# ctlab/metafast

Measured on AMD Instinct MI355X. Metric: k-mers/s counted+graphed at k=31, 150 bp reads, higher is better.
Workload: dtype u64

## Files before the change

metafast_amd/csrc/mf_common.h:

```cpp
#pragma once
#include <hip/hip_runtime.h>
#include <stdint.h>
#include <stdarg.h>
#include <stdio.h>
#include <string.h>
#include <map>
#include <string>
#include <vector>
#include "../../include/metafast_hip.h"

int mf_set_error(const char *fmt, ...);

#define MF_HIP(call)                                                                              \
    do {                                                                                          \
        hipError_t e__ = (call);                                                                  \
        if (e__ != hipSuccess)                                                                    \
            return mf_set_error("%s failed: %s (%s:%d)", #call, hipGetErrorString(e__), __FILE__, \
                                __LINE__);                                                        \
    } while (0)
#define MF_TRY(call)                  \
    do {                              \
        int r__ = (call);             \
        if (r__ < 0) return r__;      \
    } while (0)
// ... 54 lines not shown
    int64_t opt_device_parse = 1;
    int64_t opt_device_parse_piece = 8 << 20, opt_device_parse_threads = 8;
    int64_t opt_device_parse_min = 1 << 20;
    int64_t opt_host_pinned = 0;
    int64_t opt_file_cache_gb = 0;
    int64_t opt_gz_device_min = 32 << 20;
    int64_t opt_gz_piece = 2 << 20;
    int64_t opt_ut_double_after = 4;
    int64_t opt_ut_plain_rounds = 3;
    int64_t opt_cc_compress = 1;
    int64_t opt_stream_count = 1;
    int64_t opt_stream_count_min = 512 << 20, opt_stream_count_piece = 256 << 20;
    int64_t opt_stream_count_test_pct = 100;
    uint64_t n_streamed = 0, n_stream_stepped_back = 0;
    void *up_stream = nullptr;
    int64_t opt_wide_skm = 1;
    int64_t opt_wide_skm_min = 1 << 20;
    int64_t opt_wide_skm_lazy_order = 1;
    int64_t opt_wide_skm_fine = 8;
    int64_t opt_wide_skm_pack = 1;
    int64_t opt_wide_skm_merge = 1;
    int64_t opt_wide_skm_lead = 1;
    int64_t opt_wide_skm_unit = 2400;
    int64_t opt_wide_finish = 1;
    int64_t opt_wide_big_bucket = 256;
    int64_t opt_wide_distinct = 1280;
    int64_t opt_wide_ablate = 0;
    int64_t opt_wide_passes = 0;
    int64_t opt_cc_sparse = 1;
    int64_t opt_stats_slices = 0;
    int64_t opt_dcc_sparse = 0;
    int64_t opt_dcc_test_fail = 0; int64_t dcc_test_calls[3] = {0, 0, 0};
    int64_t opt_nbr_global = 0;
    int64_t opt_scatter_fast = 1;
    int64_t opt_ablate = 0;
    struct span { size_t off, sz; };
    struct region { char *base; size_t size; std::vector<span> free_spans; };
    std::vector<region> regions;
    std::vector<struct mf_file_entry *> file_cache; size_t file_cache_bytes = 0; uint64_t file_cache_clock = 0;
    size_t arena_bytes = 0;
    uint64_t n_slice_restarts = 0, n_dparse_files = 0, n_dparse_stepped_back = 0, n_wide_big = 0, n_wide_hashed = 0, n_ut_doubled = 0, n_pilots = 0, n_gz_device = 0;
    std::vector<mf_timer_rec> pending;
    std::vector<hipEvent_t> event_pool;
    struct ktime { int64_t n = 0; double total_ms = 0, max_ms = 0; };
    std::map<std::string, ktime> timings;
};

int  mf_alloc(mf_ctx *ctx, size_t bytes, void **out);
void mf_release(mf_ctx *ctx, void *p, size_t bytes);
size_t mf_arena_idle(const mf_ctx *ctx);
int  mf_collect_timers(mf_ctx *ctx);
int  mf_debug_sync(mf_ctx *ctx, const char *what);
#define MF_DBG(ctx, what) do { if ((ctx)->opt_verbose >= 2) MF_TRY(mf_debug_sync((ctx), (what))); } while (0)

struct mf_ktimer {
    mf_ctx *ctx; int idx;
    mf_ktimer(mf_ctx *c, const char *name);
    ~mf_ktimer();
};

struct mf_range {
    bool on;
    explicit mf_range(const char *name);
    ~mf_range();
};

// ... 452 lines not shown
```

metafast_amd/csrc/mf_ctx.hip:

```cpp
#include "mf_common.h"
#include <time.h>
#include <stdlib.h>

static thread_local char g_err[1024] = "";

int mf_set_error(const char *fmt, ...) {
    va_list ap;
    va_start(ap, fmt);
    vsnprintf(g_err, sizeof g_err, fmt, ap);
    va_end(ap);
    return MF_ERR;
}

extern "C" const char *mf_last_error(void) { return g_err; }

#include <dlfcn.h>
#include <mutex>
static int (*g_roctx_push)(const char *) = nullptr;
static int (*g_roctx_pop)(void) = nullptr;
static bool roctx_ready() {
    static std::once_flag once;
    std::call_once(once, [] {
        const char *want = getenv("MF_ROCTX");
        if (want ? atoi(want) == 0 : getenv("ROCP_TOOL_LIBRARIES") == nullptr) return;
// ... 155 lines not shown
    else if (s == "wide_skm_merge") ctx->opt_wide_skm_merge = v;
    else if (s == "wide_skm_pack") ctx->opt_wide_skm_pack = v;
    else if (s == "wide_skm_fine") ctx->opt_wide_skm_fine = v;
    else if (s == "wide_skm_lazy_order") ctx->opt_wide_skm_lazy_order = v;
    else if (s == "dcc_sparse") ctx->opt_dcc_sparse = v;
    else if (s == "dcc_test_fail") { ctx->opt_dcc_test_fail = v; ctx->dcc_test_calls[1] = ctx->dcc_test_calls[2] = 0; }
    else if (s == "cc_sparse") ctx->opt_cc_sparse = v;
    else if (s == "stats_slices") { if (v < 0 || v > 4096) return mf_set_error("stats_slices must be in [0, 4096]"); ctx->opt_stats_slices = v; }
    else if (s == "gz_device_min_bytes") ctx->opt_gz_device_min = v;
    else if (s == "gz_piece_bytes") { if (v < 4096) return mf_set_error("gz_piece_bytes must be at least 4096"); ctx->opt_gz_piece = v; }
    else if (s == "ut_double_after") { if (v < 1 || v > 64) return mf_set_error("ut_double_after must be in [1, 64]"); ctx->opt_ut_double_after = v; }
    else if (s == "wide_finish") ctx->opt_wide_finish = v ? 1 : 0;
    else if (s == "wide_big_bucket") { if (v < 1 || v > 256) return mf_set_error("wide_big_bucket must be in [1, 256]"); ctx->opt_wide_big_bucket = v; }
    else if (s == "wide_ablate") ctx->opt_wide_ablate = v;
    else if (s == "wide_distinct") { if (v < 1 || v > 1280) return mf_set_error("wide_distinct must be in [1, 1280]"); ctx->opt_wide_distinct = v; }
    else if (s == "wide_passes") { if (v < 0 || v > 65536) return mf_set_error("wide_passes must be in [0, 65536]"); ctx->opt_wide_passes = v; }
    else if (s == "file_cache") {
        if (v < 0) { size_t fr = 0, tot = 0; MF_HIP(hipSetDevice(ctx->device)); MF_HIP(hipMemGetInfo(&fr, &tot)); v = std::max<int64_t>(1, (int64_t)(tot >> 32) / -v); }
        ctx->opt_file_cache_gb = v;
        if (!v) mf_file_cache_clear(ctx);
    }
    else if (s == "skm_pilot") ctx->opt_skm_pilot = v;
    else if (s == "device_parse") ctx->opt_device_parse = v;
    else if (s == "device_parse_min_bytes") ctx->opt_device_parse_min = v;
    else if (s == "device_parse_piece_bytes") ctx->opt_device_parse_piece = v;
    else if (s == "device_parse_threads") ctx->opt_device_parse_threads = v;
    else if (s == "host_pinned") ctx->opt_host_pinned = v;
    else if (s == "skm_dynq") ctx->opt_skm_dynq = v;
    else if (s == "part_good") { if (v < 16 || v > 4096) return mf_set_error("part_good out of [16,4096]"); ctx->opt_part_good = v; }
    else if (s == "unit_parts_long") { if (v < 0 || v > 4) return mf_set_error("unit_parts_long out of [0,4]"); ctx->opt_unit_parts_long = v; }
    else if (s == "skm_unit_records") { if (v != 0 && (v < 64 || v > (1 << 20))) return mf_set_error("skm_unit_records out of [64,2^20] (0: by k)"); ctx->opt_skm_unit_records = v; }
    else if (s == "skm_unit_distinct") { if (v < 64 || v > 3400) return mf_set_error("skm_unit_distinct out of [64,3400]"); ctx->opt_skm_unit_distinct = v; }
    else if (s == "union_samples") ctx->opt_union_samples = v;
    else return mf_set_error("unknown option '%s'", name);
    return MF_OK;
}

extern "C" int64_t mf_ctx_stat(mf_ctx *ctx, const char *name) {
    if (!ctx || !name) return mf_set_error("mf_ctx_stat: NULL argument");
    const std::string s(name);
    if (s == "slice_restarts") return (int64_t)ctx->n_slice_restarts;
    if (s == "gz_files_inflated_into_hbm") return (int64_t)ctx->n_gz_device;
    if (s == "pilot_runs") return (int64_t)ctx->n_pilots;
    if (s == "unitig_doublings") return (int64_t)ctx->n_ut_doubled;
    if (s == "wide_big_entries") return (int64_t)ctx->n_wide_big;
    if (s == "wide_hashed_entries") return (int64_t)ctx->n_wide_hashed;
    if (s == "streamed_counts") return (int64_t)ctx->n_streamed;
    if (s == "streamed_counts_stepped_back") return (int64_t)ctx->n_stream_stepped_back;
    if (s == "device_parsed_files") return (int64_t)ctx->n_dparse_files;
    if (s == "device_parser_stepped_back") return (int64_t)ctx->n_dparse_stepped_back;
    if (s == "hipmalloc_calls") return (int64_t)ctx->n_hipmalloc;
    if (s == "hipmalloc_bytes") return (int64_t)ctx->b_hipmalloc;
    if (s == "hipmalloc_us") return (int64_t)(ctx->t_hipmalloc * 1e6);
    if (s == "arena_bytes") return (int64_t)ctx->arena_bytes;
    if (s == "arena_idle_bytes") return (int64_t)mf_arena_idle(ctx);
    return mf_set_error("mf_ctx_stat: unknown name '%s'", name);
}
extern "C" int mf_ctx_synchronize(mf_ctx *ctx) {
    if (!ctx) return mf_set_error("ctx is NULL");
    MF_HIP(hipStreamSynchronize(ctx->stream));
    return MF_OK;
}

static const size_t MF_ALIGN = 256;
static bool arena_take(mf_ctx *ctx, size_t bytes, void **out, bool spare_big) {
    int br = -1, bs = -1; size_t best = ~(size_t)0;
    for (size_t r = 0; r < ctx->regions.size(); r++)
        for (size_t s = 0; s < ctx->regions[r].free_spans.size(); s++) {
            size_t sz = ctx->regions[r].free_spans[s].sz;
            if (spare_big && sz >= ((size_t)48 << 30) && sz / 4 >= bytes) continue;
            if (sz >= bytes && sz < best) { best = sz; br = (int)r; bs = (int)s; }
        }
    if (br < 0) return false;
    auto &R = ctx->regions[br];
    mf_ctx::span sp = R.free_spans[bs];
    *out = R.base + sp.off;
// ... 133 lines not shown
```

metafast_amd/csrc/mf_skm.hip:

```cpp
#include "mf_common.h"
#include "mf_count_dev.h"
#include <algorithm>
#include <memory>
#include <vector>

typedef ulonglong2 skm_rec;
typedef uint32_t skm_v4 __attribute__((ext_vector_type(4)));
#define SKM_LINE 4
#define SKM_QCAP 16
#define SKM_DIGIT_BITS 22
#ifdef SKM_BIG_UNITS
#define SKM_CT 1024
#elif defined(SKM_SMALL_UNITS)
#define SKM_CT 256
#else
#define SKM_CT 512
#endif
#define SKM_NW (SKM_CT / 64)

__device__ __forceinline__ bool skm_rec_valid(const skm_rec &r) { return ((uint32_t)r.y & 63u) != 63u; }
__device__ __forceinline__ uint32_t skm_rec_n(const skm_rec &r) { return (uint32_t)r.y & 63u; }
__device__ __forceinline__ uint32_t skm_rec_digits(const skm_rec &r) { return (uint32_t)(r.y >> 6) & ((1u << SKM_DIGIT_BITS) - 1u); }

template <int K> struct skm_word {
// ... 188 lines not shown
};
__device__ __forceinline__ skm_stage skm_stage_carve(unsigned char *smem, int nd) {
    skm_stage L;
    L.nd = nd;
    L.line = reinterpret_cast<skm_rec *>(smem);
    L.cur = reinterpret_cast<uint64_t *>(L.line + (size_t)nd * SKM_LINE + 64);
    L.q_pos = L.cur + nd;
    L.ctr = reinterpret_cast<uint32_t *>(L.q_pos + 16 * SKM_QCAP);
    L.q_d = L.ctr + nd + 64;
    return L;
}
__host__ __device__ static inline size_t skm_stage_bytes(int nd) {
    return ((size_t)nd * SKM_LINE + 64) * 16 + (size_t)nd * 8 + 16 * SKM_QCAP * 8 + ((size_t)nd + 64) * 4 + 16 * SKM_QCAP * 4;
}
__device__ __forceinline__ void skm_lds_write4_add_rtn4(const uint32_t (&wa)[4], const skm_v4 (&wv)[4], const uint32_t (&a)[4],
                                                        const uint32_t (&inc)[4], uint32_t (&old)[4]) {
    asm volatile("ds_write_b128 %4, %8\n\tds_write_b128 %5, %9\n\tds_write_b128 %6, %10\n\tds_write_b128 %7, %11\n\t"
                 "ds_add_rtn_u32 %0, %12, %16\n\tds_add_rtn_u32 %1, %13, %17\n\tds_add_rtn_u32 %2, %14, %18\n\t"
                 "ds_add_rtn_u32 %3, %15, %19\n\ts_waitcnt lgkmcnt(0)"
                 : "=&v"(old[0]), "=&v"(old[1]), "=&v"(old[2]), "=&v"(old[3])
                 : "v"(wa[0]), "v"(wa[1]), "v"(wa[2]), "v"(wa[3]), "v"(wv[0]), "v"(wv[1]), "v"(wv[2]), "v"(wv[3]),
                   "v"(a[0]), "v"(a[1]), "v"(a[2]), "v"(a[3]), "v"(inc[0]), "v"(inc[1]), "v"(inc[2]), "v"(inc[3])
                 : "memory");
}
#define SKM_CH 256
#define SKM_NONE (~0ull)
struct skm_dyn {
    unsigned long long *gcur;
    const uint64_t *rend;
    unsigned int *overflow;
    uint64_t dump;
    unsigned long long *save;
};
template <bool DYN>
__device__ __forceinline__ uint64_t skm_take_line(const skm_stage &L, uint32_t dg, const skm_dyn &Dy) {
    uint64_t pos = L.cur[dg];
    if (DYN && (pos == SKM_NONE || (pos & (uint64_t)(SKM_CH - 1)) == 0ull)) {
        pos = atomicAdd(&Dy.gcur[dg], (unsigned long long)SKM_CH);
        if (pos + SKM_CH > Dy.rend[dg]) { atomicExch(Dy.overflow, 1u); pos = Dy.dump; }
    }
    L.cur[dg] = pos + SKM_LINE;
    return pos;
}
template <bool DYN = false>
__device__ __forceinline__ void skm_stage_insert(const skm_stage &L, skm_rec *__restrict__ out, const uint32_t (&d)[4],
                                                 const skm_rec (&rec)[4], bool (&pending)[4], const skm_dyn &Dy = skm_dyn()) {
    const uint32_t ctr0 = mf_lds_addr(L.ctr), line0 = mf_lds_addr(L.line);
    const uint32_t dummy_ctr = ctr0 + 4u * ((uint32_t)L.nd + (uint32_t)mf_lane());
    const uint32_t dummy_slot = line0 + 16u * ((uint32_t)L.nd * SKM_LINE + (uint32_t)mf_lane());
    skm_v4 wv[4];
#pragma unroll
    for (int b = 0; b < 4; b++) { wv[b].x = (uint32_t)rec[b].x; wv[b].y = (uint32_t)(rec[b].x >> 32); wv[b].z = (uint32_t)rec[b].y; wv[b].w = (uint32_t)(rec[b].y >> 32); }
    for (;;) {
        bool any = false;
#pragma unroll
        for (int b = 0; b < 4; b++) any |= pending[b];
        if (__ballot(any) == 0ull) break;
        uint32_t ca[4], w[4], inc[4], old[4], old2[4], wa[4];
        bool got[4];
#pragma unroll
        for (int b = 0; b < 4; b++) ca[b] = pending[b] ? ctr0 + 4u * d[b] : dummy_ctr;
        mf_lds_read4(ca, w);
#pragma unroll
        for (int b = 0; b < 4; b++) inc[b] = (pending[b] && (w[b] & 0xFFFFu) < (uint32_t)SKM_LINE) ? 1u : 0u;
        mf_lds_add_rtn4(ca, inc, old);
#pragma unroll
        for (int b = 0; b < 4; b++) {
            got[b] = inc[b] && (old[b] & 0xFFFFu) < (uint32_t)SKM_LINE;
            wa[b] = got[b] ? line0 + 16u * (d[b] * SKM_LINE + (old[b] & 0xFFFFu)) : dummy_slot;
            ca[b] = got[b] ? ctr0 + 4u * d[b] : dummy_ctr;
            inc[b] = got[b] ? 0x10000u : 0u;
        }
        skm_lds_write4_add_rtn4(wa, wv, ca, inc, old2);
        uint64_t *qpos = L.q_pos + (threadIdx.x >> 6) * SKM_QCAP;
        uint32_t *qd = L.q_d + (threadIdx.x >> 6) * SKM_QCAP;
        const uint64_t lt_mask = (1ull << mf_lane()) - 1ull;
#pragma unroll
        for (int b = 0; b < 4; b++) {
            const bool fl = got[b] && (old2[b] >> 16) == (uint32_t)(SKM_LINE - 1);
            const unsigned long long F = __ballot(fl);
            if (got[b]) pending[b] = false;
            if (F == 0ull) continue;
            const uint32_t n = (uint32_t)__popcll(F), qi = (uint32_t)__popcll(F & lt_mask);
            uint64_t mypos = 0;
            if (fl) mypos = skm_take_line<DYN>(L, d[b], Dy);
            for (uint32_t e0 = 0; e0 < n; e0 += SKM_QCAP) {
                if (fl && qi >= e0 && qi < e0 + SKM_QCAP) { qpos[qi - e0] = mypos; qd[qi - e0] = d[b]; }
                asm volatile("s_waitcnt lgkmcnt(0)" ::: "memory");
                const uint32_t e = e0 + ((uint32_t)mf_lane() >> 2), c = (uint32_t)mf_lane() & 3u;
                if (e < n) {
                    const uint32_t dd = qd[e - e0];
                    const uint64_t pp = qpos[e - e0];
                    const skm_rec v = L.line[dd * SKM_LINE + c];
                    out[pp + c] = v;
                    asm volatile("" ::: "memory");
                    if (c == 0) __hip_atomic_store(&L.ctr[dd], 0u, __ATOMIC_RELEASE, MF_WG);
                }
                asm volatile("s_waitcnt lgkmcnt(0)" ::: "memory");
            }
        }
        asm volatile("" ::: "memory");
        __builtin_amdgcn_wave_barrier();
    }
}
template <bool DYN = false>
__device__ __forceinline__ void skm_stage_flush_all(const skm_stage &L, skm_rec *__restrict__ out, int nd, const skm_dyn &Dy = skm_dyn()) {
    const skm_rec SENT = make_ulonglong2(~0ull, ~0ull);
    for (int d = threadIdx.x; d < nd; d += blockDim.x) {
        const uint32_t c = L.ctr[d] >> 16;
        if (c) {
            const uint64_t pos = skm_take_line<DYN>(L, (uint32_t)d, Dy);
            for (uint32_t s = 0; s < (uint32_t)SKM_LINE; s++) out[pos + s] = s < c ? L.line[d * SKM_LINE + s] : SENT;
            L.ctr[d] = 0;
        }
        if (DYN) {
            uint64_t pos = L.cur[d];
            if (Dy.save) Dy.save[(size_t)blockIdx.x * nd + d] = pos;
            else if (pos != SKM_NONE) for (; (pos & (uint64_t)(SKM_CH - 1)) != 0ull; pos++) out[pos] = SENT;
        }
    }
}
__global__ void k_skm_close_chunks(const unsigned long long *__restrict__ save, uint64_t n, uint64_t cap, skm_rec *__restrict__ out) {
    const uint64_t i = (uint64_t)blockIdx.x * blockDim.x + threadIdx.x;
    if (i >= n) return;
    uint64_t pos = save[i];
    if (pos == SKM_NONE || pos >= cap) return;
    const skm_rec SENT = make_ulonglong2(~0ull, ~0ull);
    for (; (pos & (uint64_t)(SKM_CH - 1)) != 0ull; pos++) out[pos] = SENT;
}

#define SKM_LCAP 384
#define SKM_FAST_WAVE_BYTES (64 * 16 + 64 * 8 + (SKM_LCAP + 1) * 8)
template <int K, bool DYN, bool FAST>
__global__ __launch_bounds__(1024) void k_skm_scatter(const uint8_t *__restrict__ bases, uint64_t n_bases, const uint32_t *__restrict__ vmask,
                                                      uint64_t n_words, uint64_t words_per_block, int bits1,
                                                      const uint64_t *__restrict__ blockstart, int G, skm_rec *__restrict__ out, skm_dyn Dy,
                                                      uint32_t dlo, uint32_t dhi) {
    extern __shared__ __attribute__((aligned(16))) unsigned char smem[];
    const int nd = 1 << bits1;
    skm_stage L = skm_stage_carve(smem, nd);
    if (DYN) Dy.dump += (uint64_t)blockIdx.x * SKM_CH;
    for (int i = threadIdx.x; i < nd; i += blockDim.x) {
        L.cur[i] = DYN ? (Dy.save ? (uint64_t)Dy.save[(size_t)blockIdx.x * nd + i] : SKM_NONE) : blockstart[(size_t)i * G + blockIdx.x];
        L.ctr[i] = 0;
    }
// ... 171 lines not shown
            for (int dd = 32; dd >= 1; dd >>= 1) raw += __shfl_down(raw, dd, 64);
            if (mf_lane() == 0 && raw) atomicAdd(n_valid, (unsigned long long)raw);
        }
        uint32_t tot;
        uint32_t ex = mf_block_excl_scan(mine, scratch, &tot);
        for (int j = 0; j < ipt; j++) {
            const int b = b0 + j;
            if (b < nd) {
                const uint32_t c = (L.ctr[b] + 3u) & ~3u;
                L.cur[b] = obase + ex;
                ostart[(size_t)p * nd + b] = obase + ex;
                olen[(size_t)p * nd + b] = c;
                if (oocc) oocc[(size_t)p * nd + b] = occ[b];
                ex += c;
            }
        }
        __syncthreads();
        for (int i = threadIdx.x; i < nd; i += blockDim.x) L.ctr[i] = 0;
        if (threadIdx.x < 64) L.ctr[nd + threadIdx.x] = 0;
        __syncthreads();
        for (uint32_t jb = 0; jb < len; jb += 4 * blockDim.x) {
            skm_rec v[4]; uint32_t d[4]; bool pend[4];
#pragma unroll
            for (int u = 0; u < 4; u++) {
                const uint32_t j = jb + u * blockDim.x + threadIdx.x;
                v[u] = j < len ? src[j] : make_ulonglong2(~0ull, ~0ull);
                pend[u] = skm_rec_valid(v[u]);
                d[u] = pend[u] ? ((skm_rec_digits(v[u]) >> shift) & dmask) : 0u;
            }
            skm_stage_insert(L, out, d, v, pend);
        }
        __syncthreads();
        skm_stage_flush_all(L, out, nd);
        __syncthreads();
    }
}

#define SKM_MAX_PASSES 64
__device__ __forceinline__ uint32_t skm_pass_of(uint64_t key) {
    uint32_t g = ((uint32_t)(key >> 32) * 0xC2B2AE35u) ^ ((uint32_t)key * 0x27D4EB2Fu);
    g ^= g >> 15; g *= 0x165667B1u;
    return g >> 24;
}

#ifdef SKM_BIG_UNITS
#define C2_SLOTS 8192
#define C2_FILL 6800
#define C2_WG_PER_CU 1
#elif defined(SKM_SMALL_UNITS)
#define C2_SLOTS 2048
#define C2_FILL 1700
#define C2_WG_PER_CU 3
#else
#define C2_WG_PER_CU 2
#define C2_SLOTS 4096
#define C2_FILL 3400
#endif
#define C2_QN 128
#define C2_LH 64
#define C2_ITEMS 848
#define C2_W 2
#define DD_BITS (SKM_CT > 512 ? 12 : 11)
#define C2_DD 4
static constexpr size_t C2_LDS = (size_t)C2_SLOTS * 12 + (size_t)SKM_CT * 16 + (size_t)(SKM_CT / 64) * (C2_ITEMS * 2 + C2_QN * 8 + C2_QN * 2) + 2 * C2_LH * 4 + 48;
static_assert(C2_LDS <= 160 * 1024 / C2_WG_PER_CU, "workgroups per CU");

// ... 939 lines not shown
            int Bc = 0; while (Bc < 30 && (double)(1ull << Bc) < want_units) Bc++;
            const int r = std::max(1, std::min(Bc - bits1, std::min((int)SKM_DIGIT_BITS, 30 - bits1)));
            if (ctx->opt_verbose) fprintf(stderr, "[mf] skm pilot: %.4f distinct k-mers per occurrence -> %d bits after level 1 (planned from the occurrences alone: %d)\n", rho, r, total_bits - bits1);
            lv.resize(1);
            if (r <= MF_MAX_DIGIT_BITS) lv.push_back(r); else { lv.push_back((r + 1) / 2); lv.push_back(r / 2); }
            total_bits = 0; for (int b : lv) total_bits += b;
            if (kthr >= 0 && kept >= 0.0 && !A.doff.p) {
                const double per_unit = (double)n_occ * kept / (double)(1ull << total_bits);
                int sb = 0; while (sb < 4 && per_unit / (double)(1 << sb) > (double)ctx->opt_part_good) sb++;
                A.split_bits = sb; split_from_pilot = true;
                if (ctx->opt_verbose) fprintf(stderr, "[mf] skm pilot: %.4f k-mers per occurrence survive the cut: %.0f per counting unit -> %d table partition(s) per unit\n", kept, per_unit, 1 << sb);
            }
        }
    }
    if (!A.doff.p) {
        if (!split_from_pilot) A.split_bits = A.table_bits > 0 ? std::max(0, std::min(4, A.table_bits - total_bits)) : 1;
        if (total_bits + A.split_bits > 30) A.split_bits = 30 - total_bits;
        A.np_total = (uint32_t)(1ull << (total_bits + A.split_bits));
        MF_TRY(A.doff.alloc(ctx, (size_t)A.np_total + 1));
    }
    MF_HIP(hipMemsetAsync(&scal[6], 0, 8, st));
    headroom = false;
    const unsigned long long cap_l1 = cap, cap_last = final_cap(cap);
    if (dlo != 0 || dhi != (uint32_t)nd1) {
        np = dhi - dlo;
        mf_buf<uint64_t> ps; MF_TRY(ps.alloc(ctx, np)); mf_buf<uint32_t> pl, po; MF_TRY(pl.alloc(ctx, np)); MF_TRY(po.alloc(ctx, np));
        MF_HIP(hipMemcpyAsync(ps.p, pstart.p + dlo, (size_t)np * 8, hipMemcpyDeviceToDevice, st));
        MF_HIP(hipMemcpyAsync(pl.p, plen.p + dlo, (size_t)np * 4, hipMemcpyDeviceToDevice, st));
        MF_HIP(hipMemcpyAsync(po.p, pocc.p + dlo, (size_t)np * 4, hipMemcpyDeviceToDevice, st));
        pstart.swap(ps); plen.swap(pl); pocc.swap(po);
    }
    int used = 0;
    mf_buf<skm_rec> spare;
    for (size_t li = 1; li < lv.size(); li++) {
        const int bits = lv[li], nd = 1 << bits;
        const uint64_t cap2 = cap + (uint64_t)np * SKM_LINE * nd;
        const uint64_t np2 = (uint64_t)np * nd;
        if (np2 > 0xFFFFFFF0ull) return mf_set_error("too many partitions");
        const bool last = li + 1 == lv.size();
        mf_buf<skm_rec> bufB;
        if (spare.p && spare.n >= cap2) bufB.swap(spare);
        else if (bufB.alloc(ctx, std::max<unsigned long long>(cap2, cap_last)) != MF_OK) {
            if (ctx->opt_verbose) fprintf(stderr, "[mf] skm: no room for %.1f GB of level-%zu records (arena %.1f GB): %s\n", cap2 * 16 / 1e9, li + 1, ctx->arena_bytes / 1e9, mf_last_error());
            return MF_SKM_NOMEM;
        }
        mf_buf<uint64_t> ostart; MF_TRY(ostart.alloc(ctx, np2));
        mf_buf<uint32_t> olen; MF_TRY(olen.alloc(ctx, np2));
        mf_buf<uint32_t> oocc; if (last) MF_TRY(oocc.alloc(ctx, np2));
        const size_t lds = skm_stage_bytes(nd);
        const unsigned grid = (unsigned)std::min<uint64_t>(np, (uint64_t)ctx->n_cu * (lds > 72 * 1024 ? 1 : 2));
        {
            MF_TRY(skm_set_lds(k_skm_split, lds));
            mf_ktimer t(ctx, "k_skm_split");
            k_skm_split<<<grid, 1024, lds, st>>>(bufA.p, pstart.p, plen.p, np, SKM_DIGIT_BITS - used - bits, bits, bufB.p, ostart.p, olen.p, oocc.p,
                                                 li == 1 ? &scal[6] : nullptr, li == 1 ? rebase : 0);
        }
        MF_DBG(ctx, "k_skm_split");
        if (ctx->opt_verbose >= 2 && last) {
            std::vector<uint32_t> h(np2);
            MF_HIP(hipMemcpyAsync(h.data(), olen.p, np2 * 4, hipMemcpyDeviceToHost, st));
            MF_HIP(hipStreamSynchronize(st));
            double tot = 0, tot2 = 0, mx = 0;
            for (uint32_t v : h) { tot += v; tot2 += (double)v * v; mx = std::max(mx, (double)v); }
            const double mean = tot / (double)np2, sd = std::sqrt(std::max(0.0, tot2 / (double)np2 - mean * mean));
            const double slack[4] = {0.06, 0.12, 0.25, 0.50};
            double over[4] = {0, 0, 0, 0}, parts[4] = {0, 0, 0, 0}, room[4] = {0, 0, 0, 0};
            for (uint32_t v : h) {
                const double n = v, mu = n / 16.0, sg = std::sqrt(n / 16.0 * 15.0 / 16.0);
                for (int q = 0; q < 4; q++) {
                    double e = 0, pr = 0, rm = 0;
                    for (int zi = -40; zi <= 40; zi++) {
                        const double z = zi * 0.1, w = std::exp(-0.5 * z * z) * 0.1 / 2.5066282746;
                        const double cap = std::max(0.0, 16.0 * (mu + z * sg) * (1.0 + slack[q]) + 64.0);
                        if (n > cap) { e += w * (n - cap); pr += w; }
                        rm += w * cap;
                    }
                    over[q] += e; parts[q] += pr; room[q] += rm;
                }
            }
            fprintf(stderr, "[mf] skm split, one-pass what-if: %llu sub-partitions of %.0f records on average (sd %.0f, largest %.0f); sized from a 1/16 sample + slack:\n", (unsigned long long)np2, mean, sd, mx);
            for (int q = 0; q < 4; q++)
                fprintf(stderr, "[mf]     slack %2.0f %%: %.3f %% of the records overflow (%.0f records in %.0f sub-partitions), the regions take %.2f x the records\n", slack[q] * 100.0,
                        100.0 * over[q] / std::max(tot, 1.0), over[q], parts[q], room[q] / std::max(tot, 1.0));
        }
        bufA.swap(bufB);
        if (!last && bufB.owned) { spare.reset(); spare.swap(bufB); }
        else if (!last && SH && last_of_shared && bufB.p == SH->buf.p) {
            bufB.reset(); spare.reset(); spare.swap(SH->buf); SH->ready = false;
        }
        pstart.swap(ostart); plen.swap(olen);
        if (last) pocc.swap(oocc);
        cap = cap2; np = (uint32_t)np2; used += bits;
    }

    spare.reset();
    mf_buf<uint32_t> pcap; MF_TRY(pcap.alloc(ctx, np));
    mf_buf<uint64_t> toff; MF_TRY(toff.alloc(ctx, (size_t)np + 1));
    k_skm_cap<<<(np + 255) / 256, 256, 0, st>>>(pocc.p, np, pcap.p, kthr >= 0 ? (uint32_t)kthr + 1u : 1u);
    MF_TRY(mf_scan<1>(ctx, pcap.p, toff.p, np, (uint64_t *)&scal[4]));
    uint32_t nbatch = 1;
    if (ctx->opt_skm_batches > 0) nbatch = (uint32_t)std::min<int64_t>(ctx->opt_skm_batches, np);
    else {
        unsigned long long tall = 0;
        MF_HIP(hipMemcpyAsync(&tall, &scal[4], 8, hipMemcpyDeviceToHost, st));
        MF_HIP(hipStreamSynchronize(st));
        size_t fr = 0, tot = 0;
        MF_HIP(hipMemGetInfo(&fr, &tot));
        double budget = (ctx->opt_arena_cap_gb > 0 ? (double)ctx->opt_arena_cap_gb * 1e9 : (double)tot) * 0.22;
        if (ctx->opt_arena_cap_gb <= 0) budget = std::min(budget, ((double)fr + (double)mf_arena_idle(ctx)) * 0.5);
        if (n_occ < (1ull << 32)) budget = std::min(budget, 3e9);
        while (nbatch < 64 && nbatch * 2 <= np && (double)tall * 10.0 / nbatch > budget) nbatch *= 2;
    }
    const uint32_t PB = (np + nbatch - 1) / nbatch;
// ... 66 lines not shown
            if (nk.alloc(ctx, want) != MF_OK || nc.alloc(ctx, want) != MF_OK) return MF_SKM_NOMEM;
            if (dused) {
                MF_HIP(hipMemcpyAsync(nk.p, dk.p, dused * 8, hipMemcpyDeviceToDevice, st));
                MF_HIP(hipMemcpyAsync(nc.p, dc.p, dused * 2, hipMemcpyDeviceToDevice, st));
                MF_HIP(hipStreamSynchronize(st));
            }
            dk.swap(nk); dc.swap(nc);
            dcap = want;
        }
        {
            const unsigned grid = (unsigned)std::min<uint64_t>(((uint64_t)(p1 - p0) + 3) / 4, (uint64_t)ctx->n_cu * 32);
            mf_ktimer t(ctx, "k_gather");
            if (A.split_bits == 1)
                k_gather_split<K><<<grid, 256, 0, st>>>(tkeys.p, tcnt.p, toff.p, dcount.p, coff.p, p1, dk.p + dused, dc.p + dused, p0, (uint64_t)tb[b],
                                                        doffp, dused, 31 - total_bits);
            else
                k_gather_split_n<K><<<grid, 256, 0, st>>>(tkeys.p, tcnt.p, toff.p, dcount.p, coff.p, p1, dk.p + dused, dc.p + dused, p0, (uint64_t)tb[b],
                                                          doffp, dused, std::min(31, 32 - total_bits - A.split_bits), A.split_bits);
        }
        MF_DBG(ctx, "k_gather");
        dused += d_b;
    }
    MF_HIP(hipGetLastError());
    bufA.reset();
    {
        unsigned long long nv = 0;
        MF_HIP(hipMemcpyAsync(&nv, &scal[6], 8, hipMemcpyDeviceToHost, st));
        MF_HIP(hipStreamSynchronize(st));
        A.n_records += nv ? nv : cap_l1;
    }
    if (ctx->opt_verbose)
        fprintf(stderr, "[mf] count(skm): slice %u/%u digits [%u,%u): records=%llu levels=%zu bits=%d np=%u distinct so far=%llu\n", slice + 1, n_slices, dlo, dhi,
                (unsigned long long)cap, lv.size(), total_bits, np, (unsigned long long)dused);
    return MF_OK;
}

template <int K>
static int skm_run(mf_ctx *ctx, const uint8_t *d_bases, uint64_t n_bases, const uint32_t *vmask, uint64_t n_words,
                   uint64_t n_occ, const std::vector<int> &lv0, bool adaptive, int table_bits, unsigned long long *scal, int thr, uint64_t *n_all, mf_table **out,
                   skm_shared *pre = nullptr) {
    hipStream_t st = ctx->stream;
    std::vector<int> lv = lv0;
    const int bits1 = lv[0], nd1 = 1 << bits1;
    int total_bits = 0; for (int b : lv) total_bits += b;
    if (total_bits > 30 || total_bits - bits1 > SKM_DIGIT_BITS) return MF_SKM_FALLBACK;
    const int kthr = thr < C2_LH ? thr : -1;
    MF_TRY(skm_set_lds(k_skm_count<K, false>, C2_LDS));
    if (K == 31) MF_TRY(skm_set_lds(k_skm_count<(K == 31 ? 31 : 20), true>, C2_LDS));
    uint32_t S = 1;
    bool shared = false;
    if (lv.size() >= 2) {
        size_t fr = 0, tot = 0;
        MF_HIP(hipMemGetInfo(&fr, &tot));
        if (ctx->opt_skm_slices > 0) S = (uint32_t)ctx->opt_skm_slices;
        else {
            double budget = (ctx->opt_arena_cap_gb > 0 ? (double)ctx->opt_arena_cap_gb * 1e9 : (double)tot * 0.92) - (double)n_bases * 1.15 - 8e9;
            const double table = (double)n_occ * 0.14 * 26.0;
            budget -= std::min(table, budget * 0.5);
            const double recs = (double)n_occ / 5.5 * 16.0 * 2.3;
            while (S < 64 && recs / S > budget) S *= 2;
        }
        while (S > 1 && (uint32_t)nd1 / S < 4) S /= 2;
        if (S > 1 && ctx->opt_skm_shared == 2) shared = true;
        else if (S > 1 && ctx->opt_skm_shared == 1 && ctx->opt_arena_cap_gb <= 0) {
            const double avail = ((double)fr + (double)mf_arena_idle(ctx)) * 0.96 - (double)n_occ * (kthr >= 1 ? 0.04 : 0.10) * 10.0 * 1.3 - (double)tot * 0.05;
            const double run = std::min<double>((K - mf_skm_m(K) + 2) / 2.0, (double)skm_word<K>::RMAX) * 0.78;
// ... 268 lines not shown
```

Before: 88.85 billion.

## Split super-k-mer partitions in one read using sampled sub-partition sizing with spill list

Adds a one-read split path for super-k-mer partitioning. Each partition's sub-partition ranges are sized from a strided sample plus slack, and records are written straight into those bounded ranges. Records that overflow go to a per-partition spill list and are compacted afterwards, and a partition that exhausts its spill room is redone with exact counts. The aim is to avoid reading every record twice (count then scatter) in the split. In exchange it allocates larger output buffers, adds a planning kernel and host syncs, and makes the kernel more complex with fallback paths.

```diff
diff --git a/metafast_amd/csrc/mf_common.h b/metafast_amd/csrc/mf_common.h
--- a/metafast_amd/csrc/mf_common.h
+++ b/metafast_amd/csrc/mf_common.h
@@ -110,6 +110,14 @@
     int64_t opt_dcc_sparse = 0;
     int64_t opt_dcc_test_fail = 0; int64_t dcc_test_calls[3] = {0, 0, 0};
     int64_t opt_nbr_global = 0;
+    int64_t opt_split_once = 1;
+    int64_t opt_split_sample_stride = 4;
+    int64_t opt_split_slack_pct = 20;
+    int64_t opt_split_floor = 16;
+    int64_t opt_split_spill_pct = -1;
+    int64_t opt_split_test_nofit = 0;
+    int64_t opt_split_sample_min = 256;
+    uint64_t n_split_redone = 0, n_split_moved = 0, n_split_spilled = 0, n_split_sampled = 0, n_split_sampled_sub = 0, n_split_sampled_rec = 0;
     int64_t opt_scatter_fast = 1;
     int64_t opt_ablate = 0;
     struct span { size_t off, sz; };
diff --git a/metafast_amd/csrc/mf_ctx.hip b/metafast_amd/csrc/mf_ctx.hip
--- a/metafast_amd/csrc/mf_ctx.hip
+++ b/metafast_amd/csrc/mf_ctx.hip
@@ -211,6 +211,13 @@
     else if (s == "skm_unit_records") { if (v != 0 && (v < 64 || v > (1 << 20))) return mf_set_error("skm_unit_records out of [64,2^20] (0: by k)"); ctx->opt_skm_unit_records = v; }
     else if (s == "skm_unit_distinct") { if (v < 64 || v > 3400) return mf_set_error("skm_unit_distinct out of [64,3400]"); ctx->opt_skm_unit_distinct = v; }
     else if (s == "union_samples") ctx->opt_union_samples = v;
+    else if (s == "split_once") ctx->opt_split_once = v ? 1 : 0;
+    else if (s == "split_sample_stride") { if (v < 1 || v > 1024) return mf_set_error("split_sample_stride out of [1,1024]"); ctx->opt_split_sample_stride = v; }
+    else if (s == "split_slack_pct") { if (v < 0 || v > 400) return mf_set_error("split_slack_pct out of [0,400]"); ctx->opt_split_slack_pct = v; }
+    else if (s == "split_floor") { if (v < 0 || v > 65536) return mf_set_error("split_floor out of [0,65536]"); ctx->opt_split_floor = v; }
+    else if (s == "split_spill_pct") { if (v < -1 || v > 400) return mf_set_error("split_spill_pct out of [-1,400]"); ctx->opt_split_spill_pct = v; }
+    else if (s == "split_test_nofit") ctx->opt_split_test_nofit = v ? 1 : 0;
+    else if (s == "split_sample_min") { if (v < 1 || v > (1 << 20)) return mf_set_error("split_sample_min out of [1,2^20]"); ctx->opt_split_sample_min = v; }
     else return mf_set_error("unknown option '%s'", name);
     return MF_OK;
 }
@@ -221,6 +228,12 @@
     if (s == "slice_restarts") return (int64_t)ctx->n_slice_restarts;
     if (s == "gz_files_inflated_into_hbm") return (int64_t)ctx->n_gz_device;
     if (s == "pilot_runs") return (int64_t)ctx->n_pilots;
+    if (s == "split_redone") return (int64_t)ctx->n_split_redone;
+    if (s == "split_moved") return (int64_t)ctx->n_split_moved;
+    if (s == "split_spilled_records") return (int64_t)ctx->n_split_spilled;
+    if (s == "split_sampled") return (int64_t)ctx->n_split_sampled;
+    if (s == "split_sampled_subparts") return (int64_t)ctx->n_split_sampled_sub;
+    if (s == "split_sampled_records") return (int64_t)ctx->n_split_sampled_rec;
     if (s == "unitig_doublings") return (int64_t)ctx->n_ut_doubled;
     if (s == "wide_big_entries") return (int64_t)ctx->n_wide_big;
     if (s == "wide_hashed_entries") return (int64_t)ctx->n_wide_hashed;
diff --git a/metafast_amd/csrc/mf_skm.hip b/metafast_amd/csrc/mf_skm.hip
--- a/metafast_amd/csrc/mf_skm.hip
+++ b/metafast_amd/csrc/mf_skm.hip
@@ -244,9 +244,24 @@
     uint64_t dump;
     unsigned long long *save;
 };
-template <bool DYN>
-__device__ __forceinline__ uint64_t skm_take_line(const skm_stage &L, uint32_t dg, const skm_dyn &Dy) {
+struct skm_bnd {
+    uint32_t *lim;
+    uint32_t *ovf;
+    uint32_t *sp;
+    uint32_t *occ;
+    uint64_t base, spill0;
+    uint32_t spill_cap;
+};
+template <bool DYN, bool BOUND = false>
+__device__ __forceinline__ uint64_t skm_take_line(const skm_stage &L, uint32_t dg, const skm_dyn &Dy, const skm_bnd &Bd = skm_bnd()) {
     uint64_t pos = L.cur[dg];
+    if (BOUND && (uint32_t)(pos - Bd.base) + (uint32_t)SKM_LINE > Bd.lim[dg]) {
+        if (Bd.sp[1]) return SKM_NONE;
+        const uint32_t at = atomicAdd(&Bd.sp[0], (uint32_t)SKM_LINE);
+        if (at + (uint32_t)SKM_LINE > Bd.spill_cap) { Bd.sp[1] = 1u; return SKM_NONE; }
+        Bd.ovf[dg]++;
+        return Bd.spill0 + at;
+    }
     if (DYN && (pos == SKM_NONE || (pos & (uint64_t)(SKM_CH - 1)) == 0ull)) {
         pos = atomicAdd(&Dy.gcur[dg], (unsigned long long)SKM_CH);
         if (pos + SKM_CH > Dy.rend[dg]) { atomicExch(Dy.overflow, 1u); pos = Dy.dump; }
@@ -254,9 +269,10 @@
     L.cur[dg] = pos + SKM_LINE;
     return pos;
 }
-template <bool DYN = false>
+template <bool DYN = false, bool BOUND = false>
 __device__ __forceinline__ void skm_stage_insert(const skm_stage &L, skm_rec *__restrict__ out, const uint32_t (&d)[4],
-                                                 const skm_rec (&rec)[4], bool (&pending)[4], const skm_dyn &Dy = skm_dyn()) {
+                                                 const skm_rec (&rec)[4], bool (&pending)[4], const skm_dyn &Dy = skm_dyn(),
+                                                 const skm_bnd &Bd = skm_bnd()) {
     const uint32_t ctr0 = mf_lds_addr(L.ctr), line0 = mf_lds_addr(L.line);
     const uint32_t dummy_ctr = ctr0 + 4u * ((uint32_t)L.nd + (uint32_t)mf_lane());
     const uint32_t dummy_slot = line0 + 16u * ((uint32_t)L.nd * SKM_LINE + (uint32_t)mf_lane());
@@ -295,7 +311,7 @@
             if (F == 0ull) continue;
             const uint32_t n = (uint32_t)__popcll(F), qi = (uint32_t)__popcll(F & lt_mask);
             uint64_t mypos = 0;
-            if (fl) mypos = skm_take_line<DYN>(L, d[b], Dy);
+            if (fl) mypos = skm_take_line<DYN, BOUND>(L, d[b], Dy, Bd);
             for (uint32_t e0 = 0; e0 < n; e0 += SKM_QCAP) {
                 if (fl && qi >= e0 && qi < e0 + SKM_QCAP) { qpos[qi - e0] = mypos; qd[qi - e0] = d[b]; }
                 asm volatile("s_waitcnt lgkmcnt(0)" ::: "memory");
@@ -304,7 +320,13 @@
                     const uint32_t dd = qd[e - e0];
                     const uint64_t pp = qpos[e - e0];
                     const skm_rec v = L.line[dd * SKM_LINE + c];
-                    out[pp + c] = v;
+                    if (!BOUND || pp != SKM_NONE) out[pp + c] = v;
+                    if (BOUND && Bd.occ) {
+                        uint32_t nk = skm_rec_n(v);
+                        nk += (uint32_t)__builtin_amdgcn_update_dpp(0, (int)nk, 0xB1 , 0xF, 0xF, false);
+                        nk += (uint32_t)__builtin_amdgcn_update_dpp(0, (int)nk, 0x4E , 0xF, 0xF, false);
+                        if (c == 0) atomicAdd(&Bd.occ[dd], nk);
+                    }
                     asm volatile("" ::: "memory");
                     if (c == 0) __hip_atomic_store(&L.ctr[dd], 0u, __ATOMIC_RELEASE, MF_WG);
                 }
@@ -315,14 +337,17 @@
         __builtin_amdgcn_wave_barrier();
     }
 }
-template <bool DYN = false>
-__device__ __forceinline__ void skm_stage_flush_all(const skm_stage &L, skm_rec *__restrict__ out, int nd, const skm_dyn &Dy = skm_dyn()) {
+template <bool DYN = false, bool BOUND = false>
+__device__ __forceinline__ void skm_stage_flush_all(const skm_stage &L, skm_rec *__restrict__ out, int nd, const skm_dyn &Dy = skm_dyn(),
+                                                    const skm_bnd &Bd = skm_bnd()) {
     const skm_rec SENT = make_ulonglong2(~0ull, ~0ull);
     for (int d = threadIdx.x; d < nd; d += blockDim.x) {
         const uint32_t c = L.ctr[d] >> 16;
         if (c) {
-            const uint64_t pos = skm_take_line<DYN>(L, (uint32_t)d, Dy);
-            for (uint32_t s = 0; s < (uint32_t)SKM_LINE; s++) out[pos + s] = s < c ? L.line[d * SKM_LINE + s] : SENT;
+            const uint64_t pos = skm_take_line<DYN, BOUND>(L, (uint32_t)d, Dy, Bd);
+            if (!BOUND || pos != SKM_NONE)
+                for (uint32_t s = 0; s < (uint32_t)SKM_LINE; s++) out[pos + s] = s < c ? L.line[d * SKM_LINE + s] : SENT;
+            if (BOUND && Bd.occ) { uint32_t nk = 0; for (uint32_t s = 0; s < c; s++) nk += skm_rec_n(L.line[d * SKM_LINE + s]); atomicAdd(&Bd.occ[d], nk); }
             L.ctr[d] = 0;
         }
         if (DYN) {
@@ -560,6 +585,188 @@
         }
         __syncthreads();
         skm_stage_flush_all(L, out, nd);
+        __syncthreads();
+    }
+}
+
+#define SKM_EXACT 0xFFFFFFFFu
+struct skm_once_par {
+    uint32_t stride, slack_pct, floor, min_len;
+    int32_t spill_pct;
+};
+__host__ __device__ static inline size_t skm_once_lds(int nd) { return ((skm_stage_bytes(nd) + 15) & ~(size_t)15) + (size_t)nd * 16 + 64; }
+__global__ void k_skm_split_plan(const uint32_t *__restrict__ plen, uint32_t np, int nd, skm_once_par P, uint32_t *__restrict__ pcap,
+                                 uint32_t *__restrict__ pspill, unsigned long long *__restrict__ too_big) {
+    const uint32_t p = blockIdx.x * blockDim.x + threadIdx.x;
+    const uint64_t len = p < np ? plen[p] : 0ull;
+    const unsigned long long samp = __ballot(p < np && len >= (uint64_t)P.min_len);
+    if (mf_lane() == 0 && samp) atomicAdd(&too_big[2], (unsigned long long)__popcll(samp));
+    if (p >= np) return;
+    uint64_t cap, spill;
+    if (len < (uint64_t)P.min_len) { cap = len + (uint64_t)SKM_LINE * nd; spill = SKM_EXACT; }
+    else {
+        const uint64_t area = (len + len * P.slack_pct / 100 + (uint64_t)nd * (SKM_LINE + P.floor) + 3) & ~3ull;
+        if (P.spill_pct >= 0) spill = len * (uint64_t)P.spill_pct / 100;
+        else {
+            const float n = (float)len / (float)nd, sd = sqrtf(n * (float)(P.stride - 1)) + 1e-3f;
+            const float z = (n * (float)P.slack_pct * 0.01f + (float)P.floor) / sd;
+            spill = len / 50 + (uint64_t)((float)len * 0.75f * erfcf(z * 0.70710678f)) + 64;
+        }
+        spill = (spill + 3) & ~3ull;
+        cap = area + spill;
+    }
+    if (cap > 0x7FFFFFF0ull) { atomicExch(too_big, 1ull); cap = 0; spill = SKM_EXACT; }
+    pcap[p] = (uint32_t)cap;
+    pspill[p] = (uint32_t)spill;
+}
+__global__ __launch_bounds__(1024) void k_skm_split_once(const skm_rec *__restrict__ in, const uint64_t *__restrict__ pstart,
+                                                         const uint32_t *__restrict__ plen, uint32_t np, int shift, int bits, skm_rec *out,
+                                                         const uint64_t *__restrict__ obase, const uint32_t *__restrict__ pspill,
+                                                         uint64_t *__restrict__ ostart, uint32_t *__restrict__ olen, uint32_t *__restrict__ oocc,
+                                                         unsigned long long *__restrict__ n_valid, unsigned long long *__restrict__ stat,
+                                                         uint32_t stride, uint32_t slack_pct, uint32_t floor_) {
+    extern __shared__ __attribute__((aligned(16))) unsigned char smem[];
+    __shared__ uint32_t scratch[17];
+    const int nd = 1 << bits;
+    const uint32_t dmask = (uint32_t)nd - 1u;
+    skm_stage L = skm_stage_carve(smem, nd);
+    uint32_t *lim = reinterpret_cast<uint32_t *>(smem + ((skm_stage_bytes(nd) + 15) & ~(size_t)15));
+    uint32_t *beg = lim + nd, *ovf = beg + nd, *occ = ovf + nd;
+    uint32_t *sp = occ + nd;
+    const int ipt = (nd + (int)blockDim.x - 1) / (int)blockDim.x;
+    const int b0 = threadIdx.x * ipt;
+    const uint32_t blk = 4u * blockDim.x;
+    const uint32_t lane = (uint32_t)mf_lane();
+    for (uint32_t p = blockIdx.x; p < np; p += gridDim.x) {
+        const uint32_t len = plen[p];
+        const uint64_t base = obase[p];
+        const uint32_t room = (uint32_t)(obase[p + 1] - base), spl = pspill[p];
+        const skm_rec *src = in + pstart[p];
+        uint32_t nval = 0;
+        for (int pass = spl != SKM_EXACT ? 0 : 1; pass < 2; pass++) {
+            const bool exact = pass == 1;
+            const uint32_t area = exact ? room : room - spl;
+            for (int i = threadIdx.x; i < nd; i += blockDim.x) L.ctr[i] = 0;
+            __syncthreads();
+            uint64_t ns = 0;
+            for (uint32_t jb = 0, bi = 0; jb < len; jb += blk, bi++) {
+                if (!exact && bi % stride) continue;
+                ns += len - jb < blk ? len - jb : blk;
+                skm_rec v[4];
+#pragma unroll
+                for (int u = 0; u < 4; u++) { const uint32_t j = jb + u * blockDim.x + threadIdx.x; v[u] = j < len ? src[j] : make_ulonglong2(~0ull, ~0ull); }
+#pragma unroll
+                for (int u = 0; u < 4; u++)
+                    if (skm_rec_valid(v[u])) atomicAdd(&L.ctr[(skm_rec_digits(v[u]) >> shift) & dmask], 1u);
+            }
+            __syncthreads();
+            const double scale = exact ? 1.0 : (double)len / (double)(ns ? ns : 1) * (double)(100u + slack_pct) * 0.01;
+            auto want = [&](int b) -> uint32_t {
+                const uint32_t c = L.ctr[b];
+                if (exact) return (c + 3u) & ~3u;
+                const uint64_t e = ((uint64_t)((double)c * scale) + floor_ + 3u) & ~3ull;
+                return e > (uint64_t)area ? (area & ~3u) : (uint32_t)e;
+            };
+            uint32_t mine = 0, tot;
+            for (int j = 0; j < ipt; j++) if (b0 + j < nd) mine += want(b0 + j);
+            uint32_t ex = mf_block_excl_scan(mine, scratch, &tot);
+            double shrink = 1.0;
+            if (tot > area) {
+                shrink = (double)area / (double)tot;
+                mine = 0;
+                for (int j = 0; j < ipt; j++) if (b0 + j < nd) mine += (uint32_t)((double)want(b0 + j) * shrink) & ~3u;
+                ex = mf_block_excl_scan(mine, scratch, &tot);
+            }
+            for (int j = 0; j < ipt; j++) {
+                const int b = b0 + j;
+                if (b < nd) {
+                    uint32_t c = want(b);
+                    if (shrink < 1.0) c = (uint32_t)((double)c * shrink) & ~3u;
+                    L.cur[b] = base + ex; beg[b] = ex; lim[b] = ex + c; ovf[b] = 0; occ[b] = 0;
+                    ex += c;
+                }
+            }
+            if (threadIdx.x == 0) { sp[0] = 0; sp[1] = 0; sp[2] = 0; }
+            __syncthreads();
+            for (int i = threadIdx.x; i < nd; i += blockDim.x) L.ctr[i] = 0;
+            if (threadIdx.x < 64) L.ctr[nd + threadIdx.x] = 0;
+            __syncthreads();
+            skm_bnd Bd;
+            Bd.lim = lim; Bd.ovf = ovf; Bd.sp = sp; Bd.occ = oocc ? occ : nullptr; Bd.base = base; Bd.spill0 = base + area; Bd.spill_cap = room - area;
+            nval = 0;
+            for (uint32_t jb = 0; jb < len; jb += blk) {
+                skm_rec v[4]; uint32_t d[4]; bool pend[4];
+#pragma unroll
+                for (int u = 0; u < 4; u++) {
+                    const uint32_t j = jb + u * blockDim.x + threadIdx.x;
+                    v[u] = j < len ? src[j] : make_ulonglong2(~0ull, ~0ull);
+                    pend[u] = skm_rec_valid(v[u]);
+                    d[u] = pend[u] ? ((skm_rec_digits(v[u]) >> shift) & dmask) : 0u;
+                    nval += pend[u] ? 1u : 0u;
+                }
+                skm_stage_insert<false, true>(L, out, d, v, pend, skm_dyn(), Bd);
+            }
+            __syncthreads();
+            skm_stage_flush_all<false, true>(L, out, nd, skm_dyn(), Bd);
+            __syncthreads();
+            const uint32_t listed = sp[0];
+            const bool full = sp[1] != 0u;
+            __syncthreads();
+            if (!full)
+                for (int j = 0; j < ipt; j++) {
+                    const int b = b0 + j;
+                    if (b >= nd) break;
+                    const size_t at = (size_t)p * nd + b;
+                    const uint32_t here = (uint32_t)(L.cur[b] - base) - beg[b], o = ovf[b];
+                    if (!o) { ostart[at] = base + beg[b]; olen[at] = here; }
+                    else {
+                        const uint32_t need = here + o * (uint32_t)SKM_LINE, to = atomicAdd(&sp[0], need);
+                        if ((uint64_t)to + need > (uint64_t)Bd.spill_cap) sp[1] = 1u; else lim[b] = to;
+                        atomicAdd(&sp[2], 1u);
+                    }
+                    if (oocc) oocc[at] = occ[b];
+                }
+            __syncthreads();
+            if (sp[1]) {
+                if (threadIdx.x == 0) atomicAdd(&stat[exact ? 6 : 0], 1ull);
+                continue;
+            }
+            if (sp[2]) {
+                const uint64_t lt_mask = (1ull << lane) - 1ull;
+                for (uint32_t b = threadIdx.x >> 6; b < (uint32_t)nd; b += blockDim.x >> 6) {
+                    const uint32_t o = ovf[b];
+                    if (!o) continue;
+                    const uint64_t from = base + beg[b], to = Bd.spill0 + lim[b];
+                    const uint32_t here = (uint32_t)(L.cur[b] - from);
+                    for (uint32_t i = lane; i < here; i += 64u) out[to + i] = out[from + i];
+                    uint32_t k = 0;
+                    for (uint32_t l0 = 0; l0 < listed; l0 += 64u * SKM_LINE) {
+                        const uint32_t at = l0 + lane * SKM_LINE;
+                        bool m = false;
+                        skm_rec v0 = make_ulonglong2(~0ull, ~0ull);
+                        if (at < listed) { v0 = out[Bd.spill0 + at]; m = ((skm_rec_digits(v0) >> shift) & dmask) == b; }
+                        const unsigned long long M = __ballot(m);
+                        if (m) {
+                            const uint64_t dst = to + here + (uint64_t)(k + (uint32_t)__popcll(M & lt_mask)) * SKM_LINE;
+                            out[dst] = v0;
+                            for (uint32_t s = 1; s < (uint32_t)SKM_LINE; s++) out[dst + s] = out[Bd.spill0 + at + s];
+                        }
+                        k += (uint32_t)__popcll(M);
+                    }
+                    if (lane == 0) { ostart[(size_t)p * nd + b] = to; olen[(size_t)p * nd + b] = here + o * (uint32_t)SKM_LINE; }
+                }
+            }
+            if (threadIdx.x == 0 && !exact) {
+                atomicAdd(&stat[3], 1ull); atomicAdd(&stat[4], (unsigned long long)nd); atomicAdd(&stat[5], (unsigned long long)len);
+                if (sp[2]) atomicAdd(&stat[1], (unsigned long long)sp[2]);
+                if (listed) atomicAdd(&stat[2], (unsigned long long)listed);
+            }
+            break;
+        }
+        if (n_valid) {
+            for (int dd = 32; dd >= 1; dd >>= 1) nval += __shfl_down(nval, dd, 64);
+            if (lane == 0 && nval) atomicAdd(n_valid, (unsigned long long)nval);
+        }
         __syncthreads();
     }
 }
@@ -1565,31 +1772,94 @@
     }
     int used = 0;
     mf_buf<skm_rec> spare;
+    bool once = ctx->opt_split_once != 0, gapped = false;
+    for (size_t li = 1; li < lv.size(); li++) if (skm_once_lds(1 << lv[li]) > (size_t)159 * 1024) once = false;
+    unsigned long long sst[8] = {0, 0, 0, 0, 0, 0, 0, 0};
     for (size_t li = 1; li < lv.size(); li++) {
         const int bits = lv[li], nd = 1 << bits;
-        const uint64_t cap2 = cap + (uint64_t)np * SKM_LINE * nd;
+        uint64_t cap2 = cap + (uint64_t)np * SKM_LINE * nd;
         const uint64_t np2 = (uint64_t)np * nd;
         if (np2 > 0xFFFFFFF0ull) return mf_set_error("too many partitions");
         const bool last = li + 1 == lv.size();
         mf_buf<skm_rec> bufB;
-        if (spare.p && spare.n >= cap2) bufB.swap(spare);
-        else if (bufB.alloc(ctx, std::max<unsigned long long>(cap2, cap_last)) != MF_OK) {
-            if (ctx->opt_verbose) fprintf(stderr, "[mf] skm: no room for %.1f GB of level-%zu records (arena %.1f GB): %s\n", cap2 * 16 / 1e9, li + 1, ctx->arena_bytes / 1e9, mf_last_error());
-            return MF_SKM_NOMEM;
+        mf_buf<uint32_t> pcap, pspill; mf_buf<uint64_t> obase; mf_buf<unsigned long long> sstat;
+        skm_once_par P;
+        P.stride = (uint32_t)ctx->opt_split_sample_stride; P.slack_pct = (uint32_t)ctx->opt_split_slack_pct; P.floor = (uint32_t)ctx->opt_split_floor;
+        P.spill_pct = (int32_t)ctx->opt_split_spill_pct;
+        P.min_len = (uint32_t)std::min<uint64_t>(0xFFFFFFFFull, (uint64_t)ctx->opt_split_sample_min * P.stride * (uint64_t)nd);
+        bool use_once = once;
+        if (use_once) {
+            MF_TRY(pcap.alloc(ctx, np)); MF_TRY(pspill.alloc(ctx, np)); MF_TRY(obase.alloc(ctx, (size_t)np + 1)); MF_TRY(sstat.alloc(ctx, 10));
+            for (int attempt = 0; attempt < 2 && !bufB.p; attempt++) {
+                if (attempt) P.min_len = 0xFFFFFFFFu;
+                MF_HIP(hipMemsetAsync(sstat.p, 0, 80, st));
+                k_skm_split_plan<<<(np + 255) / 256, 256, 0, st>>>(plen.p, np, nd, P, pcap.p, pspill.p, &sstat.p[7]);
+                MF_TRY(mf_scan<1>(ctx, pcap.p, obase.p, np, (uint64_t *)&scal[1]));
+                unsigned long long tot = 0, fl[3] = {0, 0, 0};
+                MF_HIP(hipMemcpyAsync(&tot, &scal[1], 8, hipMemcpyDeviceToHost, st));
+                MF_HIP(hipMemcpyAsync(fl, &sstat.p[7], 24, hipMemcpyDeviceToHost, st));
+                MF_HIP(hipStreamSynchronize(st));
+                if (fl[0] || !fl[2]) {
+                    if (!gapped) { use_once = false; break; }
+                    if (fl[0]) {
+                        if (ctx->opt_verbose) fprintf(stderr, "[mf] skm: a partition of level %zu is too large for the split's 31-bit offsets, using the k-mer path\n", li + 1);
+                        return MF_SKM_FALLBACK;
+                    }
+                }
+                if (!attempt) {
+                    size_t fr = 0, all = 0;
+                    MF_HIP(hipMemGetInfo(&fr, &all));
+                    const double extra = ((double)tot - (double)cap2) * 16.0, room = (double)fr + (double)mf_arena_idle(ctx);
+                    if (ctx->opt_split_test_nofit || (!(spare.p && spare.n >= tot) && extra > room * 0.25)) {
+                        if (ctx->opt_verbose) fprintf(stderr, "[mf] skm: %.1f GB more for the sampled split of level %zu with %.1f GB free: the level takes the two-read form\n", extra / 1e9, li + 1, room / 1e9);
+                        continue;
+                    }
+                }
+                if (spare.p && spare.n >= tot) bufB.swap(spare);
+                else if (bufB.alloc(ctx, std::max<unsigned long long>(tot, cap_last)) != MF_OK) {
+                    if (ctx->opt_verbose) fprintf(stderr, "[mf] skm: no room for %.1f GB of level-%zu records (arena %.1f GB)%s: %s\n", tot * 16 / 1e9, li + 1, ctx->arena_bytes / 1e9,
+                                                  attempt ? "" : ", the level takes the two-read split", mf_last_error());
+                    if (attempt) return MF_SKM_NOMEM;
+                    continue;
+                }
+                cap2 = tot;
+            }
+        }
+        if (!use_once) {
+            if (spare.p && spare.n >= cap2) bufB.swap(spare);
+            else if (bufB.alloc(ctx, std::max<unsigned long long>(cap2, cap_last)) != MF_OK) {
+                if (ctx->opt_verbose) fprintf(stderr, "[mf] skm: no room for %.1f GB of level-%zu records (arena %.1f GB): %s\n", cap2 * 16 / 1e9, li + 1, ctx->arena_bytes / 1e9, mf_last_error());
+                return MF_SKM_NOMEM;
+            }
         }
         mf_buf<uint64_t> ostart; MF_TRY(ostart.alloc(ctx, np2));
         mf_buf<uint32_t> olen; MF_TRY(olen.alloc(ctx, np2));
         mf_buf<uint32_t> oocc; if (last) MF_TRY(oocc.alloc(ctx, np2));
-        const size_t lds = skm_stage_bytes(nd);
+        const size_t lds = use_once ? skm_once_lds(nd) : skm_stage_bytes(nd);
         const unsigned grid = (unsigned)std::min<uint64_t>(np, (uint64_t)ctx->n_cu * (lds > 72 * 1024 ? 1 : 2));
-        {
+        if (use_once) {
+            MF_TRY(skm_set_lds(k_skm_split_once, lds));
+            mf_ktimer t(ctx, "k_skm_split");
+            k_skm_split_once<<<grid, 1024, lds, st>>>(bufA.p, pstart.p, plen.p, np, SKM_DIGIT_BITS - used - bits, bits, bufB.p, obase.p, pspill.p, ostart.p, olen.p,
+                                                      oocc.p, li == 1 ? &scal[6] : nullptr, sstat.p, P.stride, P.slack_pct, P.floor);
+            gapped = true;
+        } else {
             MF_TRY(skm_set_lds(k_skm_split, lds));
             mf_ktimer t(ctx, "k_skm_split");
             k_skm_split<<<grid, 1024, lds, st>>>(bufA.p, pstart.p, plen.p, np, SKM_DIGIT_BITS - used - bits, bits, bufB.p, ostart.p, olen.p, oocc.p,
                                                  li == 1 ? &scal[6] : nullptr, li == 1 ? rebase : 0);
         }
         MF_DBG(ctx, "k_skm_split");
-        if (ctx->opt_verbose >= 2 && last) {
+        if (use_once) {
+            unsigned long long h[8];
+            MF_HIP(hipMemcpyAsync(h, sstat.p, 64, hipMemcpyDeviceToHost, st));
+            MF_HIP(hipStreamSynchronize(st));
+            if (h[6]) return mf_set_error("k_skm_split_once: a two-read pass ran out of room");
+            for (int i = 0; i < 6; i++) sst[i] += h[i];
+            ctx->n_split_redone += h[0]; ctx->n_split_moved += h[1]; ctx->n_split_spilled += h[2];
+            ctx->n_split_sampled += h[3]; ctx->n_split_sampled_sub += h[4]; ctx->n_split_sampled_rec += h[5];
+        }
+        if (ctx->opt_verbose >= 2 && last && !use_once) {
             std::vector<uint32_t> h(np2);
             MF_HIP(hipMemcpyAsync(h.data(), olen.p, np2 * 4, hipMemcpyDeviceToHost, st));
             MF_HIP(hipStreamSynchronize(st));
@@ -1611,7 +1881,7 @@
                     over[q] += e; parts[q] += pr; room[q] += rm;
                 }
             }
-            fprintf(stderr, "[mf] skm split, one-pass what-if: %llu sub-partitions of %.0f records on average (sd %.0f, largest %.0f); sized from a 1/16 sample + slack:\n", (unsigned long long)np2, mean, sd, mx);
+            fprintf(stderr, "[mf] skm split (two reads), what a 1/16-sampled one-read split would meet: %llu sub-partitions of %.0f records on average (sd %.0f, largest %.0f); sized from a 1/16 sample + slack:\n", (unsigned long long)np2, mean, sd, mx);
             for (int q = 0; q < 4; q++)
                 fprintf(stderr, "[mf]     slack %2.0f %%: %.3f %% of the records overflow (%.0f records in %.0f sub-partitions), the regions take %.2f x the records\n", slack[q] * 100.0,
                         100.0 * over[q] / std::max(tot, 1.0), over[q], parts[q], room[q] / std::max(tot, 1.0));
@@ -1744,6 +2014,10 @@
     if (ctx->opt_verbose)
         fprintf(stderr, "[mf] count(skm): slice %u/%u digits [%u,%u): records=%llu levels=%zu bits=%d np=%u distinct so far=%llu\n", slice + 1, n_slices, dlo, dhi,
                 (unsigned long long)cap, lv.size(), total_bits, np, (unsigned long long)dused);
+    if (ctx->opt_verbose && sst[3])
+        fprintf(stderr, "[mf] skm split, one read: %llu partition(s) / %llu sub-partitions / %llu records sized from a sample; %llu sub-partition(s) moved (%.4f %%), "
+                        "%llu records through a spill list (%.4f %%), %llu partition(s) done again with exact ranges\n", sst[3], sst[4], sst[5], sst[1],
+                100.0 * (double)sst[1] / (double)sst[4], sst[2], 100.0 * (double)sst[2] / (double)std::max<unsigned long long>(1, sst[5]), sst[0]);
     return MF_OK;
 }
 
```

After: 90.38 billion (median of 5 runs). 1.02x the previous value.
